# furio1999/EO_Diffusion

Hardware: AMD Instinct MI355X
Metric: denoising steps/sec (UNet fwd + DDPM update) at 256x256 bs=16 (higher is better)
Workload: dtype f32; 1 GPU; DDPM sampling step, 256x256x3, batch 16 per GPU, UNet arch A0 (base 128, mults [1,2,3,4], 1 res-block(s), attn_res []), Philox noise, x0-clipped update; global_batch=16, image_size=256, parallelism=batch-sharded x1, accumulate=fp32, precision_mode=fp32x3

## Files before the change

### eo_diffusion_amd/csrc/igemm.hip

```cpp
#include <type_traits>

#include "common.h"

struct IgemmP {
    const char* a0;
    const char* a1;
    const char* b;
    const float* bias;
    const float* cbias;
    const char* res;
    char* y;
    long long cbias_stride;
    int N, H, W, C0, C1, Cin, Cout, KS, stride, pad, ups, pad_tl, Ho, Wo, HoWo, Heff, Weff;
    int tw_log2, th;
    int tiles_pw, tiles_pi;
    long long lda, ldb, ldc, sa0, sa1, sb0, sb1, sc0, sc1;
    int nb1, bias_mode, c_f32;
    long long M;
    int Ncols, K, taps, KT, tiles_m, tiles_n, out_nchw;
    int kc0, kc1;
    int tapmajor_log2;
    int ldk;
    const float* gn_ss;
    int gn_silu;
    float* stats;
    int stats_P, tiles_per_image;
    int splitk;
    int splitk_per;
    float alpha;
    const float* w_scale;
    const int* w_rexp;
    int w_row0;
    int Hd, Wd, HWd, par, par_y, par_x;
    unsigned taplist;
    const char* sx0;
    const char* sx1;
    const char* b2;
    int SC0, SC1, skc0, skc1;
    int n_base;
    int tpw;
    const float* a_bound;
    const float* skip_bound;
    const float* b_bound;
    int ab_tab_off;
    int a_ps;
    const float* y_ps_bound;
};

template <typename T> struct Mma;
template <> struct Mma<half_t> {
    static __device__ __forceinline__ void run(const i32x4& a, const i32x4& b, f32x16& c) {
        c = __builtin_amdgcn_mfma_f32_32x32x16_f16(__builtin_bit_cast(half8, a), __builtin_bit_cast(half8, b), c, 0, 0, 0);
    }
};
template <> struct Mma<float> {
    static __device__ __forceinline__ void run(const i32x4& a, const i32x4& b, f32x16& c) {
        f32x4 af = __builtin_bit_cast(f32x4, a), bf = __builtin_bit_cast(f32x4, b);
#pragma unroll
        for (int j = 0; j < 4; ++j) c = __builtin_amdgcn_mfma_f32_32x32x2f32(af[j], bf[j], c, 0, 0, 0);
    }
};

#define EOD_SPLIT_ASCALE 16.0f
__device__ __forceinline__ void split4(const f32x4& f, int (&hi)[2], int (&lo)[2]) {
    half4 h, l;
#pragma unroll
    for (int e = 0; e < 4; ++e) {
        h[e] = (half_t)f[e];
        l[e] = (half_t)(f[e] - (float)h[e]);
    }
    const auto hb = __builtin_bit_cast(__attribute__((ext_vector_type(2))) int, h);
    const auto lb = __builtin_bit_cast(__attribute__((ext_vector_type(2))) int, l);
    hi[0] = hb[0]; hi[1] = hb[1]; lo[0] = lb[0]; lo[1] = lb[1];
}
__device__ __forceinline__ void split4_scaled(const f32x4& v, float s, int (&hi)[2], int (&lo)[2]) {
    int h01, h23, l01, l23;
    asm("v_fma_mixlo_f16 %0, %4, %5, 0\n\t"
        "v_fma_mixlo_f16 %1, %4, %7, 0\n\t"
        "v_fma_mixhi_f16 %0, %4, %6, 0\n\t"
        "v_fma_mixhi_f16 %1, %4, %8, 0\n\t"
        "v_fma_mixlo_f16 %2, %4, %5, -%0 op_sel_hi:[0,0,1]\n\t"
        "v_fma_mixlo_f16 %3, %4, %7, -%1 op_sel_hi:[0,0,1]\n\t"
        "v_fma_mixhi_f16 %2, %4, %6, -%0 op_sel:[0,0,1] op_sel_hi:[0,0,1]\n\t"
        "v_fma_mixhi_f16 %3, %4, %8, -%1 op_sel:[0,0,1] op_sel_hi:[0,0,1]"
        : "=&v"(h01), "=&v"(h23), "=&v"(l01), "=&v"(l23)
        : "v"(s), "v"(v[0]), "v"(v[1]), "v"(v[2]), "v"(v[3]));
    hi[0] = h01; hi[1] = h23; lo[0] = l01; lo[1] = l23;
}
__device__ __forceinline__ i32x4 split_pair_exchange_scaled(const f32x4& v, float s, bool odd_chunk) {
    int hi[2], lo[2];
    split4_scaled(v, s, hi, lo);
    const int s0 = odd_chunk ? hi[0] : lo[0], s1 = odd_chunk ? hi[1] : lo[1];
    const int r0 = __builtin_amdgcn_mov_dpp(s0, 0xB1, 0xF, 0xF, true), r1 = __builtin_amdgcn_mov_dpp(s1, 0xB1, 0xF, 0xF, true);
    return odd_chunk ? i32x4{r0, r1, lo[0], lo[1]} : i32x4{hi[0], hi[1], r0, r1};
}
__device__ __forceinline__ i32x4 split_pair_exchange(const f32x4& f, bool odd_chunk) {
    int hi[2], lo[2];
    split4(f, hi, lo);
    const int s0 = odd_chunk ? hi[0] : lo[0], s1 = odd_chunk ? hi[1] : lo[1];
    const int r0 = __builtin_amdgcn_mov_dpp(s0, 0xB1, 0xF, 0xF, true), r1 = __builtin_amdgcn_mov_dpp(s1, 0xB1, 0xF, 0xF, true);
    return odd_chunk ? i32x4{r0, r1, lo[0], lo[1]} : i32x4{hi[0], hi[1], r0, r1};
}

typedef __attribute__((address_space(3))) void lds_void;

#define EOD_OOB 0x80000000u
#define EOD_WINDOW 0x80000000u

__device__ __forceinline__ __amdgpu_buffer_rsrc_t make_rsrc(const void* base) {
    return __builtin_amdgcn_make_buffer_rsrc(const_cast<void*>(base), 0, (int)EOD_WINDOW, 0x00020000);
}
__device__ __forceinline__ void blds16(__amdgpu_buffer_rsrc_t rs, unsigned voff, unsigned soff, char* lds_dst_wave_uniform) {
    __builtin_amdgcn_raw_ptr_buffer_load_lds(rs, (lds_void*)lds_dst_wave_uniform, 16, voff, soff, 0, 0);
}

struct TileGeom {
    int tile_m, n_first, rem_first, ty0, tx0;
    long long offA, offB, offC;
};

template <int BM>
__device__ __forceinline__ bool decode_row(const IgemmP& p, const TileGeom& g, int r, int& nrel, int& ho, int& wo) {
    if (p.tw_log2 >= 0) {
        nrel = 0;
        ho = g.ty0 + (r >> p.tw_log2);
        wo = g.tx0 + (r & ((1 << p.tw_log2) - 1));
        const bool inside = wo < p.Wd;
        if (p.par) {
            ho = 2 * ho + p.par_y;
            wo = 2 * wo + p.par_x;
        }
        return inside;
    }
    int rem = g.rem_first + r;
    nrel = 0;
    if (rem >= p.HWd) {
        nrel = rem / p.HWd;
        rem -= nrel * p.HWd;
    }
    ho = rem / p.Wd;
    wo = rem - ho * p.Wd;
    if (p.par) {
        ho = 2 * ho + p.par_y;
        wo = 2 * wo + p.par_x;
    }
    return (long long)g.tile_m * BM + r < p.M;
}

template <bool CONV, int BM>
__device__ __forceinline__ TileGeom make_geom(const IgemmP& p, int tile_m) {
    TileGeom g = {};
    g.tile_m = tile_m;
    if constexpr (CONV) {
        if (p.tw_log2 >= 0) {
            g.n_first = tile_m / p.tiles_pi;
            const int t = tile_m - g.n_first * p.tiles_pi;
            const int ty = t / p.tiles_pw;
            g.ty0 = ty * p.th;
            g.tx0 = (t - ty * p.tiles_pw) << p.tw_log2;
        } else {
            const long long m0 = (long long)tile_m * BM;
            g.n_first = (int)(m0 / p.HWd);
            g.rem_first = (int)(m0 - (long long)g.n_first * p.HWd);
        }
    } else {
        const int z = blockIdx.y;
        const int b0 = z / p.nb1, b1 = z - b0 * p.nb1;
        g.offA = b0 * p.sa0 + b1 * p.sa1;
        g.offB = b0 * p.sb0 + b1 * p.sb1;
        g.offC = b0 * p.sc0 + b1 * p.sc1;
    }
    return g;
}

#ifdef EOD_STAMP
__device__ unsigned long long g_eod_stamp[65536][16];
#define EOD_STAMP_AT(k)                                                                    \
    do {                                                                                   \
// ... 706 lines not shown
            for (int i = 0; i < TM; ++i)
#pragma unroll
                for (int j = 0; j < TN; ++j)
                    acc[i][j] = DIRECT ? __builtin_amdgcn_mfma_f32_16x16x32_f16(__builtin_bit_cast(half8, bl[j]), __builtin_bit_cast(half8, ah[i]), acc[i][j], 0, 0, 0)
                                       : __builtin_amdgcn_mfma_f32_16x16x32_f16(__builtin_bit_cast(half8, ah[i]), __builtin_bit_cast(half8, bl[j]), acc[i][j], 0, 0, 0);
#pragma unroll
            for (int i = 0; i < TM; ++i)
#pragma unroll
                for (int j = 0; j < TN; ++j)
                    acc[i][j] = DIRECT ? __builtin_amdgcn_mfma_f32_16x16x32_f16(__builtin_bit_cast(half8, bh[j]), __builtin_bit_cast(half8, ah[i]), acc[i][j], 0, 0, 0)
                                       : __builtin_amdgcn_mfma_f32_16x16x32_f16(__builtin_bit_cast(half8, ah[i]), __builtin_bit_cast(half8, bh[j]), acc[i][j], 0, 0, 0);
            continue;
        } else if constexpr (MS == 16) {
#pragma unroll
            for (int s = 0; s < 2; ++s) {
                const int o = ((4 * s + lh) ^ sw) * 16;
                i32x4 fa16[TM], fb16[TN];
#pragma unroll
                for (int i = 0; i < TM; ++i) fa16[i] = *reinterpret_cast<const i32x4*>(sb + a_rd + i * MS * BKB + o);
#pragma unroll
                for (int j = 0; j < TN; ++j) fb16[j] = *reinterpret_cast<const i32x4*>(sb + b_rd + j * MS * BKB + o);
#pragma unroll
                for (int i = 0; i < TM; ++i)
#pragma unroll
                    for (int j = 0; j < TN; ++j)
                        acc[i][j] = __builtin_amdgcn_mfma_f32_16x16x32_f16(__builtin_bit_cast(half8, fa16[i]), __builtin_bit_cast(half8, fb16[j]), acc[i][j], 0, 0, 0);
            }
            continue;
        }
        if constexpr (MS == 32) {
        i32x4 fa[2][TM], fb[2][TN];
#pragma unroll
        for (int i = 0; i < TM; ++i) fa[0][i] = *reinterpret_cast<const i32x4*>(sb + a_rd + i * 32 * BKB + coff[0]);
#pragma unroll
        for (int j = 0; j < TN; ++j) fb[0][j] = *reinterpret_cast<const i32x4*>(sb + b_rd + j * 32 * BKB + coff[0]);
        __builtin_amdgcn_sched_group_barrier(0x100, TM + TN, 0);
#pragma unroll
        for (int s = 0; s < 4; ++s) {
            const int cur = s & 1, nx = cur ^ 1;
            if (s < 3) {
#pragma unroll
                for (int i = 0; i < TM; ++i) fa[nx][i] = *reinterpret_cast<const i32x4*>(sb + a_rd + i * 32 * BKB + coff[s + 1]);
#pragma unroll
                for (int j = 0; j < TN; ++j) fb[nx][j] = *reinterpret_cast<const i32x4*>(sb + b_rd + j * 32 * BKB + coff[s + 1]);
                __builtin_amdgcn_sched_group_barrier(0x100, TM + TN, 0);
            }
#pragma unroll
            for (int i = 0; i < TM; ++i)
#pragma unroll
                for (int j = 0; j < TN; ++j) Mma<T>::run(fa[cur][i], fb[cur][j], acc[i][j]);
            __builtin_amdgcn_sched_group_barrier(0x008, TM * TN * (sizeof(T) == 4 ? 4 : 1), 0);
        }
        }
    }
    __builtin_amdgcn_s_waitcnt(0xc07f);
    __builtin_amdgcn_s_barrier();

    if constexpr (DIRECT) {
        halo_epilogue_direct<BM, BN, WAVES_M, WAVES_N>(pe, g, acc, wave, lane, n0, pre_bq, pe.alpha, pre_we);
    } else if constexpr (sizeof(T) == 4) {
        igemm_epilogue<T, CONV, BM, BN, WAVES_M, WAVES_N, true, MS>(pe, g, acc, smem, wave, lane, n0, rowtab, rowtab_n);
    } else {
        if (CONV ? p.splitk > 1 : p.c_f32 != 0)
            igemm_epilogue<T, CONV, BM, BN, WAVES_M, WAVES_N, true, MS>(pe, g, acc, smem, wave, lane, n0);
        else
            igemm_epilogue<T, CONV, BM, BN, WAVES_M, WAVES_N, false, MS>(pe, g, acc, smem, wave, lane, n0);
    }
}

template <int TN, int MS>
__device__ __forceinline__ void prefetch_bcol(const IgemmP& p, int ncols, int col0, int lane, int n_first, float (&out)[TN]) {
    const int lr = AccLayout<MS>::col(lane);
#pragma unroll
    for (int j = 0; j < TN; ++j) {
        const int col = col0 + j * MS + lr;
        const bool ok = col < ncols;
        float v = (ok && p.bias && p.bias_mode == 1) ? p.bias[col] : 0.0f;
        if (ok && p.cbias) v += p.cbias[(long long)n_first * p.cbias_stride + col];
        out[j] = v;
    }
}

template <typename T, int BN, int WAVES_M, int WAVES_N, bool UPS, int BSTAGES, bool GN, bool SPLIT = false, int MS = 32, bool SKIP = false, bool STREAM = false,
          bool KSPLIT = false>
__global__ __launch_bounds__(64 * WAVES_M * WAVES_N, WAVES_N == 4 ? 1 : 2) void conv3x3_halo_kernel(const IgemmP p) {
    static_assert(!KSPLIT || (!STREAM && !UPS && BN == 128), "K slices: the 128-column 4-wave instances");
    static_assert(!SKIP || (MS == 16 && !UPS && WAVES_M == 2), "fused skip conv: 16x16x32 instances of the 8x16 tile");
    static_assert(!SPLIT || (sizeof(T) == 4 && MS == 16), "the split-fp16 product is a mode of fp32 storage, on 16x16x32 MFMAs");
    static_assert(MS == 32 || SPLIT || sizeof(T) == 2, "the 16x16x32 shape exists for the fp16 products only");
    constexpr bool XF = GN || SPLIT;
    constexpr bool DIRECT = SPLIT && MS == 16 && BN >= 64;
    static_assert(!STREAM || (DIRECT && !SKIP && !UPS), "streaming instances: direct epilogue, no fused skip phase");
    constexpr int NW = WAVES_M * WAVES_N;
    constexpr int BM = WAVES_N == 4 ? 64 * WAVES_M : 32 * NW, TH = BM / 16, TW = 16;
    constexpr int PH = UPS ? TH / 2 + 2 : TH + 2, PW = UPS ? TW / 2 + 2 : TW + 2, PR = PH * PW;
    constexpr int PG = (PR + 7) / 8;
    constexpr int LAH = (PG + NW - 1) / NW;
    constexpr int ES = sizeof(T), EPC = 16 / ES, BKB = 128, BK = BKB / ES;
    constexpr int WM = BM / WAVES_M, WN = BN / WAVES_N, TM = WM / MS, TN = WN / MS;
    constexpr int GB = BN / 8, LB = GB / NW;
    constexpr int ABUF = PG * 1024, BSTAGE = BN * BKB;
    static_assert(GB % NW == 0 && LAH <= 6 && BSTAGES == 2, "layout");

    extern __shared__ __attribute__((aligned(16))) char smem[];
    char* const sA = smem;
    char* const sB = smem + 2 * ABUF;
    char* const sS = sB + BSTAGES * BSTAGE;
    EOD_STAMP_AT(0);

    const int tid = threadIdx.x, lane = tid & 63;
    const int wave = __builtin_amdgcn_readfirstlane(tid >> 6);
    const int wm = wave / WAVES_N, wn = wave % WAVES_N;
    int tile_m, tile_n;
    map_tile(p, tile_m, tile_n);
    int ntile = 1;
    if constexpr (STREAM) {
        tile_m *= p.tpw;
        ntile = min(p.tpw, p.tiles_m - tile_m);
    }
    const int n0 = p.n_base + tile_n * BN;
    TileGeom g = make_geom<true, BM>(p, tile_m);
    float pre_bcol[DIRECT ? 1 : TN];
    f32x4 pre_bq[DIRECT ? TN : 1];
    int pre_we[DIRECT ? TN : 1];
    if constexpr (DIRECT) {
        prefetch_bcol4<TN>(p, p.Ncols, n0 + wn * WN, lane, g.n_first, pre_bq);
        prefetch_wexp4<TN>(p, p.Ncols, n0 + wn * WN, p.w_row0, lane, pre_we);
    } else {
        prefetch_bcol<TN, MS>(p, p.Ncols, n0 + wn * WN, lane, g.n_first, pre_bcol);
    }
    float wsc1 = 1.0f;
    if constexpr (SPLIT) wsc1 = p.w_scale[1];
    AbScale asc = {EOD_SPLIT_ASCALE, 1.0f};
    const float silu_k = p.gn_silu ? -1.44269504088896341f : 0.0f, silu_c = p.gn_silu ? 0.0f : -__builtin_inff();
    if constexpr (SPLIT) {
        if (p.a_bound) asc = ab_scale_of(ab_wave_bound(p.a_bound, g.n_first));
        if constexpr (SKIP) {
            if (p.skip_bound) {
                const AbScale k = ab_scale_of(ab_wave_bound(p.skip_bound, g.n_first));
                if (k.s < asc.s) asc = k;
            }
        }
    }

    const int srow = lane >> 3, sslot = lane & 7;
    unsigned ppix[LAH];
    const int bchunk0 = sslot ^ ((4 * wave + (srow >> 1)) & 7);
    unsigned pck = 0;
    unsigned pvalid = 0;
#pragma unroll
    for (int i = 0; i < LAH; ++i) {
        const int prow = (wave + NW * i) * 8 + srow;
        const int px = prow - (prow / PW) * PW;
        pck |= (unsigned)(sslot ^ ((px >> 1) & 7)) << (3 * i);
    }
    auto set_tile_pieces = [&](const TileGeom& tg) {
        pvalid = 0;
#pragma unroll
        for (int i = 0; i < LAH; ++i) {
            const int prow = (wave + NW * i) * 8 + srow;
            const int py = prow / PW, px = prow - py * PW;
            const int hi = (UPS ? tg.ty0 / 2 : tg.ty0) - 1 + py, wi = (UPS ? tg.tx0 / 2 : tg.tx0) - 1 + px;
            const bool ok = (wave + NW * i) < PG && prow < PR && (unsigned)hi < (unsigned)p.H && (unsigned)wi < (unsigned)p.W;
            if (ok) pvalid |= 1u << i;
            ppix[i] = (unsigned)(hi * p.W + wi);
        }
    };
    set_tile_pieces(g);
    auto pchunk_of = [&](int i) { return (int)((pck >> (3 * i)) & 7u); };
    unsigned b_v[LB];
#pragma unroll
    for (int i = 0; i < LB; ++i) {
        const int row = (wave + NW * i) * 8 + srow;
        b_v[i] = (n0 + row < p.Ncols) ? (unsigned)(row * p.Cin * ES) + bchunk0 * 16 : EOD_OOB;
    }
    const __amdgpu_buffer_rsrc_t rsA0 = make_rsrc(p.a0 + (long long)g.n_first * p.H * p.W * p.C0 * ES);
    const __amdgpu_buffer_rsrc_t rsA1 = make_rsrc(p.a1 ? p.a1 + (long long)g.n_first * p.H * p.W * p.C1 * ES : p.a0);
    const __amdgpu_buffer_rsrc_t rsB = make_rsrc(p.b + (long long)n0 * p.Cin * ES);
    const int tapstride = p.Cout * p.Cin * ES;
    __amdgpu_buffer_rsrc_t rsS = rsB;
    if constexpr (GN)
        rsS = __builtin_amdgcn_make_buffer_rsrc(const_cast<float*>(p.gn_ss) + (long long)g.n_first * p.Cin * 2, 0, p.Cin * 8, 0x00020000);

    struct Chunk {
        int src, kin, cw;
// ... 130 lines not shown
    if constexpr (MS == 16) {
        constexpr int LROW = WM / 16;
        static_assert(LROW % 2 == 0, "the UPS row split needs an even first tile row per wave");
        const int c0 = SPLIT ? 2 * ((0x2130 >> (4 * lh)) & 3) : lh, c1 = SPLIT ? c0 + 1 : 4 + lh;
#pragma unroll
        for (int dx = 0; dx < 3; ++dx) {
            const int pxc = UPS ? ((lr + dx + 1) >> 1) : lr + dx;
            const int key = (pxc >> 1) & 7;
            const int rowb = ((UPS ? (wm * LROW) >> 1 : wm * LROW) * PW + pxc) * BKB;
            acur[0][dx] = rowb + ((c0 ^ key) << 4);
            acur[1][dx] = rowb + ((c1 ^ key) << 4);
        }
    }

    const int KC = p.kc0 + p.kc1;
    int kc_begin = 0, kc_end = KC;
    if constexpr (KSPLIT) {
        kc_begin = (int)blockIdx.y * p.splitk_per;
        kc_end = (int)blockIdx.y == p.splitk - 1 ? KC : kc_begin + p.splitk_per;
    }
    const int NSTEP = (kc_end - kc_begin) * 9;
    const int TSTEP = NSTEP * ntile;
    {
        const Chunk c0 = chunk_of(kc_begin);
#pragma unroll
        for (int i = 0; i < LAH; ++i)
            if ((wave + NW * i) < PG) issue_patch_piece(i, c0, sA);
        if constexpr (GN) {
            if (wave == 0) issue_ss(c0, sS);
        }
        issue_weights(0, c0, sB);
        if constexpr (XF) {
            asm volatile("s_waitcnt vmcnt(0)" ::: "memory");
            if constexpr (GN) __builtin_amdgcn_s_barrier();
#pragma unroll
            for (int i = 0; i < LAH; ++i)
                if ((wave + NW * i) < PG) transform_piece(i, c0, sA, sS);
            __builtin_amdgcn_s_waitcnt(0xc07f);
        }
    }
    EOD_STAMP_AT(1);
    int pp1 = 0;
    int step = 0;
    int qpar = 0;
    for (int k = 0; k < ntile; ++k) {
    for (int cc = kc_begin; cc < kc_end; ++cc) {
        const Chunk cur = chunk_of(cc);
        const bool next_tile = STREAM && cc + 1 == kc_end && k + 1 < ntile;
        const bool has_next = cc + 1 < kc_end || next_tile;
        const Chunk nxt = chunk_of(cc + 1 < kc_end ? cc + 1 : (next_tile ? 0 : cc));
        if constexpr (STREAM) {
            if (next_tile) set_tile_pieces(make_geom<true, BM>(p, tile_m + k + 1));
        }
        const char* abuf = sA + qpar * ABUF;
        char* abuf_next = sA + (qpar ^ 1) * ABUF;
        weight_offsets(cur, bve);
#pragma unroll
        for (int t = 0; t < 9; ++t, ++step) {
            EOD_TSTAMP_AT(4 * t + 0);
            if (!(STREAM && t == 0 && cc == kc_begin && k > 0)) {
                if (pp1 == 0) asm volatile("s_waitcnt vmcnt(0)" ::: "memory");
                else if (pp1 == 1) asm volatile("s_waitcnt vmcnt(1)" ::: "memory");
                else asm volatile("s_waitcnt vmcnt(2)" ::: "memory");
                if constexpr (XF) __builtin_amdgcn_s_waitcnt(0xc07f);
                __builtin_amdgcn_s_barrier();
            }
            EOD_TSTAMP_AT(4 * t + 1);
            if (step + 1 < TSTEP) {
                if (t < 8) issue_weights_at(t + 1, cur, bve, sB + ((step + 1) & 1) * BSTAGE);
                else issue_weights(0, nxt, sB + ((step + 1) & 1) * BSTAGE);
            }
            pp1 = 0;
            if (t < LAH && has_next && (wave + NW * t) < PG) {
                issue_patch_piece(t, nxt, abuf_next);
                pp1 = 1;
            }
            if constexpr (GN) {
                if (t == 0 && has_next && wave == 0) {
                    issue_ss(nxt, sS + (qpar ^ 1) * 1024);
                    ++pp1;
                }
            }
            EOD_TSTAMP_AT(4 * t + 2);
            const int dy = t / 3, dx = t - dy * 3;
            const char* bst = sB + (step & 1) * BSTAGE;
            int arow[TM], asw[TM];
#pragma unroll
            for (int i = 0; i < TM; ++i) {
                const int pxc = UPS ? ((pxo[i] + dx + 1) >> 1) : pxo[i] + dx;
                const int prow = UPS ? ((pyo[i] + dy + 1) >> 1) * PW + pxc : prow0[i] + dy * PW + dx;
                arow[i] = prow * BKB;
                asw[i] = (pxc >> 1) & 7;
            }
            if constexpr (MS == 16 && SPLIT) {
                const int ch = 2 * ((0x2130 >> (4 * lh)) & 3);
                i32x4 ah[TM], al[TM], bh[TN], bl[TN];
#pragma unroll
                for (int i = 0; i < TM; ++i) al[i] = *reinterpret_cast<const i32x4*>(sA + acur[1][dx] + aimm(i, dy));
#pragma unroll
                for (int j = 0; j < TN; ++j) bh[j] = *reinterpret_cast<const i32x4*>(bst + b_rd + j * MS * BKB + ((ch ^ bsw) << 4));
#pragma unroll
                for (int i = 0; i < TM; ++i) ah[i] = *reinterpret_cast<const i32x4*>(sA + acur[0][dx] + aimm(i, dy));
#pragma unroll
                for (int i = 0; i < TM; ++i)
#pragma unroll
                    for (int j = 0; j < TN; ++j)
                        acc[i][j] = DIRECT ? __builtin_amdgcn_mfma_f32_16x16x32_f16(__builtin_bit_cast(half8, bh[j]), __builtin_bit_cast(half8, al[i]), acc[i][j], 0, 0, 0)
                                           : __builtin_amdgcn_mfma_f32_16x16x32_f16(__builtin_bit_cast(half8, al[i]), __builtin_bit_cast(half8, bh[j]), acc[i][j], 0, 0, 0);
#pragma unroll
                for (int j = 0; j < TN; ++j) bl[j] = *reinterpret_cast<const i32x4*>(bst + b_rd + j * MS * BKB + (((ch + 1) ^ bsw) << 4));
#pragma unroll
                for (int i = 0; i < TM; ++i)
#pragma unroll
                    for (int j = 0; j < TN; ++j)
                        acc[i][j] = DIRECT ? __builtin_amdgcn_mfma_f32_16x16x32_f16(__builtin_bit_cast(half8, bl[j]), __builtin_bit_cast(half8, ah[i]), acc[i][j], 0, 0, 0)
                                           : __builtin_amdgcn_mfma_f32_16x16x32_f16(__builtin_bit_cast(half8, ah[i]), __builtin_bit_cast(half8, bl[j]), acc[i][j], 0, 0, 0);
#pragma unroll
                for (int i = 0; i < TM; ++i)
#pragma unroll
                    for (int j = 0; j < TN; ++j)
                        acc[i][j] = DIRECT ? __builtin_amdgcn_mfma_f32_16x16x32_f16(__builtin_bit_cast(half8, bh[j]), __builtin_bit_cast(half8, ah[i]), acc[i][j], 0, 0, 0)
                                           : __builtin_amdgcn_mfma_f32_16x16x32_f16(__builtin_bit_cast(half8, ah[i]), __builtin_bit_cast(half8, bh[j]), acc[i][j], 0, 0, 0);
            } else if constexpr (MS == 16) {
#pragma unroll
                for (int s = 0; s < 2; ++s) {
                    const int ch = 4 * s + lh;
                    i32x4 fa16[TM], fb16[TN];
#pragma unroll
                    for (int i = 0; i < TM; ++i) fa16[i] = *reinterpret_cast<const i32x4*>(sA + acur[s][dx] + aimm(i, dy));
#pragma unroll
                    for (int j = 0; j < TN; ++j) fb16[j] = *reinterpret_cast<const i32x4*>(bst + b_rd + j * MS * BKB + ((ch ^ bsw) << 4));
#pragma unroll
                    for (int i = 0; i < TM; ++i)
#pragma unroll
                        for (int j = 0; j < TN; ++j)
                            acc[i][j] = __builtin_amdgcn_mfma_f32_16x16x32_f16(__builtin_bit_cast(half8, fa16[i]), __builtin_bit_cast(half8, fb16[j]), acc[i][j], 0, 0, 0);
                }
            } else {
            i32x4 fa[2][TM], fb[2][TN];
#pragma unroll
            for (int i = 0; i < TM; ++i)
                fa[0][i] = *reinterpret_cast<const i32x4*>(abuf + arow[i] + (((0 + lh) ^ asw[i]) << 4));
#pragma unroll
            for (int j = 0; j < TN; ++j) fb[0][j] = *reinterpret_cast<const i32x4*>(bst + b_rd + j * 32 * BKB + bcoff[0]);
            __builtin_amdgcn_sched_group_barrier(0x100, TM + TN, 0);
#pragma unroll
            for (int s = 0; s < 4; ++s) {
                const int cur = s & 1, nx = cur ^ 1;
                if (s < 3) {
#pragma unroll
                    for (int i = 0; i < TM; ++i)
                        fa[nx][i] = *reinterpret_cast<const i32x4*>(abuf + arow[i] + (((2 * (s + 1) + lh) ^ asw[i]) << 4));
#pragma unroll
                    for (int j = 0; j < TN; ++j)
                        fb[nx][j] = *reinterpret_cast<const i32x4*>(bst + b_rd + j * 32 * BKB + bcoff[s + 1]);
                    __builtin_amdgcn_sched_group_barrier(0x100, TM + TN, 0);
                }
#pragma unroll
                for (int i = 0; i < TM; ++i)
#pragma unroll
                    for (int j = 0; j < TN; ++j) Mma<T>::run(fa[cur][i], fb[cur][j], acc[i][j]);
                __builtin_amdgcn_sched_group_barrier(0x008, TM * TN * (sizeof(T) == 4 ? 4 : 1), 0);
            }
            }
            EOD_TSTAMP_AT(4 * t + 3);
            if constexpr (XF) {
                if (t >= 2 && t - 2 < LAH && has_next && (wave + NW * (t - 2)) < PG)
                    transform_piece(t - 2, nxt, abuf_next, sS + (qpar ^ 1) * 1024);
            }
        }
        EOD_TSTAMP_AT(36);
#ifdef EOD_TSTAMP
        if (GN && wave == 1 && cc == 1 && k == 0 && blockIdx.x < 2048) {
            __builtin_amdgcn_s_waitcnt(0xc07f);
            if (lane < 37) g_eod_tstamp[blockIdx.x][lane] = reinterpret_cast<const unsigned long long*>(sA + ABUF + PR * 128)[lane];
        }
#endif
        if constexpr (MS == 16) {
            const int flip = qpar ? -ABUF : ABUF;
#pragma unroll
            for (int dx = 0; dx < 3; ++dx) {
                acur[0][dx] += flip;
                acur[1][dx] += flip;
            }
        }
        qpar ^= 1;
    }
    if constexpr (SKIP) {
      if (!KSPLIT || (int)blockIdx.y == p.splitk - 1) {
        constexpr int LA = BM / 8 / NW;
        constexpr int STG_A = BM * BKB, STG = STG_A + BSTAGE;
        static_assert(2 * STG <= 2 * ABUF + BSTAGES * BSTAGE, "the skip phase reuses the operand ring");
        __builtin_amdgcn_s_waitcnt(0xc07f);
        __builtin_amdgcn_s_barrier();
        const int SC = p.SC0 + p.SC1;
        const __amdgpu_buffer_rsrc_t rsX0 = make_rsrc(p.sx0 + (long long)g.n_first * p.H * p.W * p.SC0 * ES);
        const __amdgpu_buffer_rsrc_t rsX1 = make_rsrc(p.sx1 ? p.sx1 + (long long)g.n_first * p.H * p.W * p.SC1 * ES : p.sx0);
        const __amdgpu_buffer_rsrc_t rsW2 = make_rsrc(p.b2 + (long long)n0 * SC * ES);
        unsigned xpix[LA], wv[LB];
        unsigned xok = 0;
#pragma unroll
        for (int i = 0; i < LA; ++i) {
            const int row = (wave + NW * i) * 8 + srow;
            xpix[i] = (unsigned)((g.ty0 + (row >> 4)) * p.W + g.tx0 + (row & 15));
            if (g.tx0 + (row & 15) < p.W) xok |= 1u << i;
        }
#pragma unroll
        for (int i = 0; i < LB; ++i) {
            const int row = (wave + NW * i) * 8 + srow;
            wv[i] = (n0 + row < p.Ncols) ? (unsigned)(row * SC * ES) + bchunk0 * 16 : EOD_OOB;
        }
        auto issue_skip = [&](int kt, char* stg) {
            const int src = kt >= p.skc0 ? 1 : 0;
            const int kin = (src ? kt - p.skc0 : kt) * BK, cw = src ? p.SC1 : p.SC0;
            const bool ktail = kin + BK > cw;
#pragma unroll
            for (int i = 0; i < LA; ++i) {
                unsigned v = ((xok >> i) & 1u) ? xpix[i] * (unsigned)(cw * ES) + bchunk0 * 16 : EOD_OOB;
                if (ktail) v = (kin + bchunk0 * EPC < cw) ? v : EOD_OOB;
                if (src)
                    blds16(rsX1, v, (unsigned)(kin * ES), stg + (wave + NW * i) * 1024);
                else
                    blds16(rsX0, v, (unsigned)(kin * ES), stg + (wave + NW * i) * 1024);
            }
#pragma unroll
            for (int i = 0; i < LB; ++i) {
                unsigned v = wv[i];
                if (ktail) v = (kin + (SPLIT ? (bchunk0 >> 1) * 8 : bchunk0 * EPC) < cw) ? v : EOD_OOB;
                blds16(rsW2, v, (unsigned)(((src ? p.SC0 : 0) + kin) * ES), stg + STG_A + (wave + NW * i) * 1024);
            }
        };
        const int KS = p.skc0 + p.skc1;
        const int a_rd = (wm * WM + lr) * BKB;
        const int b_rd2 = STG_A + (wn * WN + lr) * BKB;
        if (KS > 0) issue_skip(0, smem);
        for (int kt = 0; kt < KS; ++kt) {
            char* stg = smem + (kt & 1) * STG;
            asm volatile("s_waitcnt vmcnt(0)" ::: "memory");
            if constexpr (SPLIT) {
#pragma unroll
                for (int i = 0; i < LA; ++i) {
                    char* ptr = stg + (wave + NW * i) * 1024 + lane * 16;
                    const f32x4 f = *reinterpret_cast<const f32x4*>(ptr);
                    *reinterpret_cast<i32x4*>(ptr) = split_pair_exchange_scaled(f, asc.s, (bchunk0 & 1) != 0);
                }
                __builtin_amdgcn_s_waitcnt(0xc07f);
            }
            __builtin_amdgcn_s_barrier();
            if (kt + 1 < KS) issue_skip(kt + 1, smem + ((kt + 1) & 1) * STG);
            if constexpr (SPLIT) {
                const int ch = 2 * ((0x2130 >> (4 * lh)) & 3);
// ... 1035 lines not shown
    EOD_CHECK_LAUNCH("conv_head");
    return EOD_OK;
}

template <typename T>
__global__ void splitk_reduce_kernel(const float* __restrict__ ws, int S, long long M, int Cout, int HoWo, float alpha,
                                     const float* __restrict__ bias, const float* __restrict__ cbias, long long cbias_stride,
                                     const T* __restrict__ res, T* __restrict__ y, const float* __restrict__ w_scale) {
    if (w_scale) alpha *= w_scale[1];
    const long long total4 = M * Cout / 4;
    for (long long i = (long long)blockIdx.x * blockDim.x + threadIdx.x; i < total4; i += (long long)gridDim.x * blockDim.x) {
        const long long e = i * 4, m = e / Cout;
        const int c = (int)(e - m * Cout);
        f32x4 a = {0.f, 0.f, 0.f, 0.f};
        for (int z = 0; z < S; ++z) a += *reinterpret_cast<const f32x4*>(ws + (long long)z * M * Cout + e);
        const long long n = m / HoWo;
#pragma unroll
        for (int k = 0; k < 4; ++k) {
            float v = a[k] * alpha;
            if (bias) v += bias[c + k];
            if (cbias) v += cbias[n * cbias_stride + c + k];
            if (res) v += (float)res[e + k];
            y[e + k] = (T)v;
        }
    }
}

template <typename T>
__global__ __launch_bounds__(256) void splitk_reduce_stats_kernel(const float* __restrict__ ws, int S, long long M, int Cout, int HoWo, float alpha,
                                                                  const float* __restrict__ bias, const float* __restrict__ cbias,
                                                                  long long cbias_stride, const T* __restrict__ res, T* __restrict__ y,
                                                                  float* __restrict__ stats) {
    __shared__ float red[16][16][8];
    const int tx = threadIdx.x & 15, ty = threadIdx.x >> 4, n = blockIdx.y;
    const int c = (blockIdx.x * 16 + tx) * 4;
    float ss[4] = {0.f, 0.f, 0.f, 0.f}, sq[4] = {0.f, 0.f, 0.f, 0.f};
    if (c < Cout) {
        float b4[4];
#pragma unroll
        for (int k = 0; k < 4; ++k) b4[k] = (bias ? bias[c + k] : 0.0f) + (cbias ? cbias[(long long)n * cbias_stride + c + k] : 0.0f);
        const long long zs = M * Cout;
        for (int pix = ty; pix < HoWo; pix += 16) {
            const long long e = ((long long)n * HoWo + pix) * Cout + c;
            f32x4 a = {0.f, 0.f, 0.f, 0.f};
            int z = 0;
            for (; z + 4 <= S; z += 4) {
                const f32x4 v0 = *reinterpret_cast<const f32x4*>(ws + (long long)z * zs + e), v1 = *reinterpret_cast<const f32x4*>(ws + (long long)(z + 1) * zs + e);
                const f32x4 v2 = *reinterpret_cast<const f32x4*>(ws + (long long)(z + 2) * zs + e), v3 = *reinterpret_cast<const f32x4*>(ws + (long long)(z + 3) * zs + e);
                a += v0; a += v1; a += v2; a += v3;
            }
            for (; z < S; ++z) a += *reinterpret_cast<const f32x4*>(ws + (long long)z * zs + e);
#pragma unroll
            for (int k = 0; k < 4; ++k) {
                float v = a[k] * alpha + b4[k];
                if (res) v += (float)res[e + k];
                const T o = (T)v;
                y[e + k] = o;
                const float x = (float)o;
                ss[k] += x;
                sq[k] += x * x;
            }
        }
    }
#pragma unroll
    for (int k = 0; k < 4; ++k) {
        red[ty][tx][2 * k] = ss[k];
        red[ty][tx][2 * k + 1] = sq[k];
    }
    __syncthreads();
    if (ty == 0 && c < Cout) {
        float* dst = stats + ((long long)n * Cout + c) * 2;
#pragma unroll
        for (int k = 0; k < 8; ++k) {
            float t = 0.0f;
#pragma unroll
            for (int r = 0; r < 16; ++r) t += red[r][tx][k];
            dst[k] = t;
        }
    }
}

#include <stdlib.h>
#include <string.h>
enum { OPT_SKIP_FUSE, OPT_HEAD, OPT_HALO_BN256, OPT_GN_FUSE_MAX_COUT, OPT_HALO_TPW, OPT_HALO_SPLITK, OPT_FIRST, OPT_HEAD_TPW, OPT_S2_HALO, OPT_COUNT };
static const char* const g_opt_name[OPT_COUNT] = {"skip_fuse", "head", "halo_bn256", "gn_fuse_max_cout", "halo_tpw", "halo_splitk", "first", "head_tpw",
                                                  "s2_halo"};
static const char* const g_opt_env[OPT_COUNT] = {"EOD_SKIP_FUSE", "EOD_HEAD", "EOD_HALO_BN256", "EOD_GN_FUSE_MAX_COUT", "EOD_HALO_TPW", "EOD_HALO_SPLITK",
                                                 "EOD_FIRST", "EOD_HEAD_TPW", "EOD_S2_HALO"};
static int g_opt[OPT_COUNT] = {1, 1, 1, -1, 1, 1, 1, 0, 1};
static bool g_opt_init = false;
static int opt(int k) {
    if (!g_opt_init) {
        for (int i = 0; i < OPT_COUNT; ++i) {
            const char* e = getenv(g_opt_env[i]);
            if (e) g_opt[i] = atoi(e);
        }
        g_opt_init = true;
    }
    return g_opt[k];
}
extern "C" int eod_set_option(const char* name, int value) {
    (void)opt(0);
    for (int i = 0; name && i < OPT_COUNT; ++i)
        if (!strcmp(name, g_opt_name[i])) {
            const int prev = g_opt[i];
            g_opt[i] = value;
            return prev;
        }
    eod_set_error("set_option: unknown option '%s'", name ? name : "(null)");
    return EOD_EINVAL;
}
extern "C" int eod_get_option(const char* name) {
    (void)opt(0);
    for (int i = 0; name && i < OPT_COUNT; ++i)
        if (!strcmp(name, g_opt_name[i])) return g_opt[i];
    eod_set_error("get_option: unknown option '%s'", name ? name : "(null)");
    return EOD_EINVAL;
}

template <typename T, bool CONV, int BM, int BN, int WAVES_M, int WAVES_N, int STAGES, bool SPLIT = false, int MS = 32, bool DIRECT = false>
static int launch_cfg(IgemmP& p, int batch, hipStream_t st) {
    constexpr int BK = 128 / (int)sizeof(T);
    constexpr int WM = BM / WAVES_M, WN = BN / WAVES_N, NW = WAVES_M * WAVES_N;
    const size_t ring = STAGES * (size_t)(BM + BN) * 128;
    const size_t epi = NW * (size_t)WM * (WN + 4) * sizeof(float);
    size_t lds = ring > epi ? ring : epi;
    if (SPLIT && CONV) {
        lds = (lds + 15) & ~(size_t)15;
        p.ab_tab_off = (int)lds;
        lds += (BM + 2) * 2 * sizeof(float);
    }
    auto kern = igemm_kernel<T, CONV, BM, BN, WAVES_M, WAVES_N, STAGES, SPLIT, MS, DIRECT>;
    static bool attr_done = false;
    if (!attr_done) {
        (void)hipFuncSetAttribute(reinterpret_cast<const void*>(kern), hipFuncAttributeMaxDynamicSharedMemorySize, (int)lds);
        attr_done = true;
    }
    if (CONV) {
        p.kc0 = (p.C0 + BK - 1) / BK;
        p.kc1 = (p.C1 + BK - 1) / BK;
        p.KT = (p.kc0 + p.kc1) * p.taps;
        if (p.tapmajor_log2 >= 0) p.KT = (9 * p.C0 + BK - 1) / BK;
    } else {
        p.KT = (p.K + BK - 1) / BK;
    }
    p.tiles_n = (p.Ncols + BN - 1) / BN;
    p.tw_log2 = -1;
    if (CONV) {
        int tw = 16;
        while (tw > p.Wd) tw >>= 1;
        if (tw >= 4 && p.Wd % tw == 0 && (BM % tw) == 0 && p.Hd % (BM / tw) == 0) {
            int l = 0;
            while ((1 << l) < tw) ++l;
            p.tw_log2 = l;
            p.th = BM / tw;
            p.tiles_pw = p.Wd / tw;
            p.tiles_pi = p.tiles_pw * (p.Hd / p.th);
            p.tiles_m = p.tiles_pi * p.N;
        } else {
            p.tiles_m = (int)((p.M + BM - 1) / BM);
        }
    } else {
        p.tiles_m = (int)((p.M + BM - 1) / BM);
    }
    const long long nblk = (long long)p.tiles_m * p.tiles_n;
    if (nblk <= 0 || nblk > 0x7fffffffLL) {
        eod_set_error("igemm: bad grid %lld", nblk);
        return EOD_EINVAL;
    }
    hipLaunchKernelGGL(kern, dim3((unsigned)nblk, (unsigned)batch), dim3(64 * NW), lds, st, p);
    EOD_CHECK_LAUNCH("igemm");
    return EOD_OK;
}

template <typename T, int BN, int WAVES_M, int WAVES_N, bool UPS, int BSTAGES, bool GN, bool SPLIT = false, int MS = 32, bool SKIP = false, bool STREAM = false,
          bool KSPLIT = false>
static int launch_halo(IgemmP& p, hipStream_t st) {
    if constexpr (!KSPLIT && !STREAM && !UPS && BN == 128 && WAVES_N == 2) {
        if (p.splitk > 1) return launch_halo<T, BN, WAVES_M, WAVES_N, UPS, BSTAGES, GN, SPLIT, MS, SKIP, false, true>(p, st);
    }
    if constexpr (!KSPLIT) {
        if (p.splitk > 1) {
            eod_set_error("conv_halo: K slices exist for the 128-column 4-wave instances only");
            return EOD_EINVAL;
        }
    }
    constexpr int BK = 128 / (int)sizeof(T);
    constexpr int NW = WAVES_M * WAVES_N, BM = WAVES_N == 4 ? 64 * WAVES_M : 32 * NW, TH = BM / 16;
    constexpr int WM = BM / WAVES_M, WN = BN / WAVES_N;
    constexpr int PR = UPS ? (TH / 2 + 2) * 10 : (TH + 2) * 18, PG = (PR + 7) / 8;
    const size_t ring = 2 * (size_t)(PG * 1024) + BSTAGES * (size_t)BN * 128 + (GN ? 2048 : 0);
    const size_t epi = NW * (size_t)WM * (WN + 4) * sizeof(float);
    const size_t lds = ring > epi ? ring : epi;
    auto kern = conv3x3_halo_kernel<T, BN, WAVES_M, WAVES_N, UPS, BSTAGES, GN, SPLIT, MS, SKIP, STREAM, KSPLIT>;
    if constexpr (SKIP) {
        p.skc0 = (p.SC0 + BK - 1) / BK;
        p.skc1 = (p.SC1 + BK - 1) / BK;
    }
    static bool attr_done = false;
    if (!attr_done) {
        (void)hipFuncSetAttribute(reinterpret_cast<const void*>(kern), hipFuncAttributeMaxDynamicSharedMemorySize, (int)lds);
        attr_done = true;
    }
    p.kc0 = (p.C0 + BK - 1) / BK;
    p.kc1 = (p.C1 + BK - 1) / BK;
    p.KT = (p.kc0 + p.kc1) * 9;
    p.tiles_n = (p.Ncols - p.n_base + BN - 1) / BN;
    p.tw_log2 = 4;
    p.th = TH;
    p.tiles_pw = (p.Wo + 15) / 16;
    p.tiles_pi = p.tiles_pw * (p.Ho / TH);
    p.tiles_m = p.tiles_pi * p.N;
    p.tiles_per_image = p.tiles_pi;
    p.tpw = 1;
    if constexpr (SPLIT && MS == 16 && BN >= 128 && !SKIP && !UPS) {
        const long long slots = 256LL * (NW == 4 ? 2 : 1);
        int want = opt(OPT_HALO_TPW);
        if (want <= 0) {
            want = 1;
            while (want < 8 && (long long)p.tiles_m * p.tiles_n / (2 * want) >= 2 * slots) want *= 2;
        }
        while (want > 1 && p.tiles_pi % want) --want;
        if (p.splitk > 1) want = 1;
        if constexpr (!STREAM) {
            if (want > 1) return launch_halo<T, BN, WAVES_M, WAVES_N, UPS, BSTAGES, GN, SPLIT, MS, SKIP, true>(p, st);
        } else {
            p.tpw = want;
        }
    }
    const long long nblk = (long long)(p.tiles_m / p.tpw) * p.tiles_n;
    if (nblk <= 0 || nblk > 0x7fffffffLL) {
        eod_set_error("conv_halo: bad grid %lld", nblk);
        return EOD_EINVAL;
    }
    hipLaunchKernelGGL(kern, dim3((unsigned)nblk, (unsigned)(p.splitk > 1 ? p.splitk : 1)), dim3(64 * NW), lds, st, p);
    EOD_CHECK_LAUNCH("conv3x3_halo");
    return EOD_OK;
}

template <typename T, bool CONV> static int launch_T(IgemmP& p, int batch, hipStream_t st) {
    if constexpr (sizeof(T) == 2) {
        if (p.Ncols <= 32) return launch_cfg<T, CONV, 128, 32, 4, 1, 2, false, 16>(p, batch, st);
        if (p.Ncols <= 64) return launch_cfg<T, CONV, 128, 64, 4, 1, 2, false, 16>(p, batch, st);
        return launch_cfg<T, CONV, 128, 128, 2, 2, 2, false, 16>(p, batch, st);
    } else {
        if (p.Ncols <= 32) return launch_cfg<T, CONV, 128, 32, 4, 1, 2>(p, batch, st);
        if (p.Ncols <= 64) return launch_cfg<T, CONV, 128, 64, 4, 1, 2>(p, batch, st);
        return launch_cfg<T, CONV, 128, 128, 2, 2, 2>(p, batch, st);
    }
}

static int launch_conv_split(IgemmP& p, int batch, hipStream_t st) {
    if (p.Ncols <= 32) return launch_cfg<float, true, 128, 32, 4, 1, 2, true, 16>(p, batch, st);
    if (p.Ncols <= 64) return launch_cfg<float, true, 128, 64, 4, 1, 2, true, 16>(p, batch, st);
    const bool direct = p.splitk <= 1 && !p.out_nchw && p.HWd % 128 == 0 && p.M % 128 == 0 && !p.par && p.Ncols % 4 == 0;
    if (p.Ncols % 256 == 0 && batch == 1 && ((p.M + 127) / 128) * (p.Ncols / 256) >= 256 && opt(OPT_HALO_BN256))
        return direct ? launch_cfg<float, true, 128, 256, 2, 4, 2, true, 16, true>(p, batch, st)
                      : launch_cfg<float, true, 128, 256, 2, 4, 2, true, 16>(p, batch, st);
    return direct ? launch_cfg<float, true, 128, 128, 2, 2, 2, true, 16, true>(p, batch, st)
                  : launch_cfg<float, true, 128, 128, 2, 2, 2, true, 16>(p, batch, st);
}

extern "C" int eod_conv_tapmajor_ldk(int C0, int dtype) {
    const int bk = 128 / (dtype == EOD_F16 ? 2 : 4);
    return (9 * C0 + bk - 1) / bk * bk;
}

static bool conv_uses_halo(const eod_conv_desc* d, int Ho, int Wo) {
    const bool shape_ok = ((d->Cout > 64 && !d->out_nchw_f32) || (d->Cout <= 32 && d->out_nchw_f32 && !d->upsample)) && d->upsample != 2;
    const bool w_ok = Wo % 16 == 0 || (Wo == 8 && d->Cout > 64 && !d->out_nchw_f32 && !d->upsample);
    return d->ksize == 3 && d->stride == 1 && d->pad == 1 && !d->pad_tl && w_ok && Ho % 8 == 0 && shape_ok && !d->w_tapmajor;
}
static int conv_waves_m(const eod_conv_desc* d, bool halo) { return (halo || d->Cout > 64) ? 2 : 4; }
static int conv_bm(const eod_conv_desc* d, bool halo) { return 128; }

static bool conv_split_ok(const eod_conv_desc* d, int Ho, int Wo) {
    return d->dtype == EOD_F32 && (d->w_tapmajor || (d->C0 % 8 == 0 && d->C1 % 8 == 0)) && d->upsample != 2;
}
static bool conv_parity_ok(const eod_conv_desc* d, int Ho, int Wo) {
    return d->upsample == 2 && d->ksize == 3 && d->stride == 1 && d->pad == 1 && !d->pad_tl && !d->out_nchw_f32 && !d->stats &&
           !d->w_tapmajor && !d->w_split && Ho % 2 == 0 && Wo % 2 == 0;
}
static bool conv_up4_ok(const eod_conv_desc* d) {
    const bool store_ok = d->dtype == EOD_F16 || (d->dtype == EOD_F32 && d->w_split);
    return d->upsample == 3 && d->ksize == 3 && d->stride == 1 && d->pad == 1 && !d->pad_tl && d->C1 == 0 && !d->x2 && d->Cout > 64 &&
           d->Cout % 8 == 0 && d->C0 % 8 == 0 && (d->W % 16 == 0 || d->W == 8) && d->H % 8 == 0 && !d->out_nchw_f32 && !d->w_tapmajor &&
           !d->gn_scale_shift && store_ok;
}
extern "C" int eod_conv_up4_ok(const eod_conv_desc* d) { return d && conv_up4_ok(d) ? 1 : 0; }
static bool conv_up4_bwd_ok(const eod_conv_desc* d) {
    return d->upsample == 4 && d->dtype == EOD_F16 && d->ksize == 3 && d->stride == 1 && d->pad == 1 && !d->pad_tl && d->C1 == 0 && !d->x2 &&
           d->Cout > 64 && d->Cout % 8 == 0 && d->C0 % 8 == 0 && d->H % 2 == 0 && d->W % 2 == 0 && d->Ho == d->H / 2 && d->Wo == d->W / 2 &&
           d->Wo % 16 == 0 && d->Ho % 8 == 0 && !d->out_nchw_f32 && !d->w_tapmajor && !d->gn_scale_shift && !d->stats && !d->w_split;
}
extern "C" int eod_conv_up4_bwd_ok(const eod_conv_desc* d) { return d && conv_up4_bwd_ok(d) ? 1 : 0; }
static int conv_up4_bwd(const eod_conv_desc* d, void* stream) {
    EOD_REQUIRE(d->N > 0 && d->H > 0 && d->W > 0 && d->C0 > 0 && d->Cout > 0 && d->x && d->w && d->y, "conv (upsample 4): bad args");
    EOD_REQUIRE(conv_up4_bwd_ok(d), "conv: upsample = 4 needs a geometry for which eod_conv_up4_bwd_ok(d) == 1");
    EOD_REQUIRE(eod_aligned16(d->x) && eod_aligned16(d->w), "conv: 16-byte alignment");
    EOD_REQUIRE((long long)d->H * d->W * d->C0 * 2 < 0x7fffffffLL && 9LL * d->Cout * 4 * d->C0 * 2 < 0x7fffffffLL, "conv (upsample 4): operand exceeds the 2 GiB window");
    IgemmP p = {};
    p.a0 = (const char*)d->x; p.b = (const char*)d->w; p.bias = d->bias; p.bias_mode = d->bias ? 1 : 0;
    p.cbias = d->cbias; p.cbias_stride = d->cbias_stride; p.res = (const char*)d->res; p.y = (char*)d->y;
    p.N = d->N; p.H = d->Ho; p.W = d->Wo;
    p.C0 = d->C0; p.C1 = 0; p.Cin = d->C0; p.Cout = d->Cout; p.KS = 3; p.stride = 1; p.pad = 1;
    p.Ho = d->Ho; p.Wo = d->Wo; p.HoWo = d->Ho * d->Wo; p.Heff = d->Ho; p.Weff = d->Wo;
    p.Hd = d->Ho; p.Wd = d->Wo; p.HWd = d->Ho * d->Wo;
    p.M = (long long)d->N * d->Ho * d->Wo; p.Ncols = d->Cout; p.taps = 9; p.alpha = d->alpha; p.nb1 = 1; p.tapmajor_log2 = -1;
// ... 426 lines not shown
```

Baseline: 39.88 steps/s.

## Interleave GroupNorm-SiLU patch transform with MFMAs via inline asm in halo conv

Adds a hand-scheduled inline-assembly block that interleaves the GroupNorm scale/shift, SiLU (exp/rcp) and fp16 hi/lo split of the next patch with the 16x16x32 MFMA chain of the current tap. Previously this transform ran after the MFMA loop. The block is enabled by default through a new option for the GN-fused split-fp32 halo instances with 64x64 wave tiles. The goal is to hide the VALU transform latency under matrix-core work. The costs are more template instances and register pressure, plus a fixed s_nop and asm volatile that constrain compiler scheduling.

```diff
diff --git a/eo_diffusion_amd/csrc/igemm.hip b/eo_diffusion_amd/csrc/igemm.hip
--- a/eo_diffusion_amd/csrc/igemm.hip
+++ b/eo_diffusion_amd/csrc/igemm.hip
@@ -87,13 +87,55 @@
         : "v"(s), "v"(v[0]), "v"(v[1]), "v"(v[2]), "v"(v[3]));
     hi[0] = h01; hi[1] = h23; lo[0] = l01; lo[1] = l23;
 }
+__device__ __forceinline__ i32x4 pair_exchange(const int (&hi)[2], const int (&lo)[2], bool odd_chunk) {
+    const int s0 = odd_chunk ? hi[0] : lo[0], s1 = odd_chunk ? hi[1] : lo[1];
+    const int r0 = __builtin_amdgcn_mov_dpp(s0, 0xB1, 0xF, 0xF, true), r1 = __builtin_amdgcn_mov_dpp(s1, 0xB1, 0xF, 0xF, true);
+    return odd_chunk ? i32x4{r0, r1, lo[0], lo[1]} : i32x4{hi[0], hi[1], r0, r1};
+}
 __device__ __forceinline__ i32x4 split_pair_exchange_scaled(const f32x4& v, float s, bool odd_chunk) {
     int hi[2], lo[2];
     split4_scaled(v, s, hi, lo);
-    const int s0 = odd_chunk ? hi[0] : lo[0], s1 = odd_chunk ? hi[1] : lo[1];
-    const int r0 = __builtin_amdgcn_mov_dpp(s0, 0xB1, 0xF, 0xF, true), r1 = __builtin_amdgcn_mov_dpp(s1, 0xB1, 0xF, 0xF, true);
-    return odd_chunk ? i32x4{r0, r1, lo[0], lo[1]} : i32x4{hi[0], hi[1], r0, r1};
-}
+    return pair_exchange(hi, lo, odd_chunk);
+}
+#define EOD_HALO_ASM_BLOCK(MIXHI, MIXLO)                  \
+    "v_fma_f32 %4, %18, %19, %20\n\t"                     \
+    "v_fma_f32 %5, %4, %21, %22\n\t"                      \
+    "v_mfma_f32_16x16x32_f16 %0, %8, %16, %0\n\t"         \
+    "v_exp_f32 %5, %5\n\t"                                \
+    "v_mfma_f32_16x16x32_f16 %1, %9, %16, %1\n\t"         \
+    "v_add_f32 %5, 1.0, %5\n\t"                           \
+    "v_mfma_f32_16x16x32_f16 %2, %10, %16, %2\n\t"        \
+    "v_rcp_f32 %5, %5\n\t"                                \
+    "v_mfma_f32_16x16x32_f16 %3, %11, %16, %3\n\t"        \
+    "v_mul_f32 %5, %4, %5\n\t"                            \
+    "v_mfma_f32_16x16x32_f16 %0, %12, %17, %0\n\t"        \
+    MIXHI "\n\t"                                          \
+    "v_mfma_f32_16x16x32_f16 %1, %13, %17, %1\n\t"        \
+    MIXLO "\n\t"                                          \
+    "v_mfma_f32_16x16x32_f16 %2, %14, %17, %2\n\t"        \
+    "v_mfma_f32_16x16x32_f16 %3, %15, %17, %3\n\t"        \
+    "v_mfma_f32_16x16x32_f16 %0, %8, %17, %0\n\t"         \
+    "v_mfma_f32_16x16x32_f16 %1, %9, %17, %1\n\t"         \
+    "v_mfma_f32_16x16x32_f16 %2, %10, %17, %2\n\t"        \
+    "v_mfma_f32_16x16x32_f16 %3, %11, %17, %3\n\t"        \
+    "s_nop 7"
+template <bool ODD>
+__device__ __forceinline__ void halo_asm_block(f32x4 (&acc)[4], const i32x4 (&bh)[4], const i32x4 (&bl)[4], const i32x4& al, const i32x4& ah,
+                                               float x, float sc, float sh, float k, float c, float s, int& hi, int& lo) {
+    float t0, t1;
+    if constexpr (ODD) {
+        asm volatile(EOD_HALO_ASM_BLOCK("v_fma_mixhi_f16 %6, %23, %5, 0", "v_fma_mixhi_f16 %7, %23, %5, -%6 op_sel:[0,0,1] op_sel_hi:[0,0,1]")
+                     : "+v"(acc[0]), "+v"(acc[1]), "+v"(acc[2]), "+v"(acc[3]), "=&v"(t0), "=&v"(t1), "+v"(hi), "+v"(lo)
+                     : "v"(bh[0]), "v"(bh[1]), "v"(bh[2]), "v"(bh[3]), "v"(bl[0]), "v"(bl[1]), "v"(bl[2]), "v"(bl[3]), "v"(al), "v"(ah),
+                       "v"(x), "v"(sc), "v"(sh), "s"(k), "v"(c), "v"(s));
+    } else {
+        asm volatile(EOD_HALO_ASM_BLOCK("v_fma_mixlo_f16 %6, %23, %5, 0", "v_fma_mixlo_f16 %7, %23, %5, -%6 op_sel_hi:[0,0,1]")
+                     : "+v"(acc[0]), "+v"(acc[1]), "+v"(acc[2]), "+v"(acc[3]), "=&v"(t0), "=&v"(t1), "=&v"(hi), "=&v"(lo)
+                     : "v"(bh[0]), "v"(bh[1]), "v"(bh[2]), "v"(bh[3]), "v"(bl[0]), "v"(bl[1]), "v"(bl[2]), "v"(bl[3]), "v"(al), "v"(ah),
+                       "v"(x), "v"(sc), "v"(sh), "s"(k), "v"(c), "v"(s));
+    }
+}
+#undef EOD_HALO_ASM_BLOCK
 __device__ __forceinline__ i32x4 split_pair_exchange(const f32x4& f, bool odd_chunk) {
     int hi[2], lo[2];
     split4(f, hi, lo);
@@ -966,7 +1008,7 @@
 }
 
 template <typename T, int BN, int WAVES_M, int WAVES_N, bool UPS, int BSTAGES, bool GN, bool SPLIT = false, int MS = 32, bool SKIP = false, bool STREAM = false,
-          bool KSPLIT = false>
+          bool KSPLIT = false, bool HASM = false>
 __global__ __launch_bounds__(64 * WAVES_M * WAVES_N, WAVES_N == 4 ? 1 : 2) void conv3x3_halo_kernel(const IgemmP p) {
     static_assert(!KSPLIT || (!STREAM && !UPS && BN == 128), "K slices: the 128-column 4-wave instances");
     static_assert(!SKIP || (MS == 16 && !UPS && WAVES_M == 2), "fused skip conv: 16x16x32 instances of the 8x16 tile");
@@ -985,6 +1027,7 @@
     constexpr int GB = BN / 8, LB = GB / NW;
     constexpr int ABUF = PG * 1024, BSTAGE = BN * BKB;
     static_assert(GB % NW == 0 && LAH <= 6 && BSTAGES == 2, "layout");
+    static_assert(!HASM || (GN && SPLIT && DIRECT && !UPS && TM == 4 && TN == 4), "halo_asm: fp32x3 GroupNorm-fused 64 x 64 wave tiles");
 
     extern __shared__ __attribute__((aligned(16))) char smem[];
     char* const sA = smem;
@@ -1281,6 +1324,8 @@
                 }
             }
             EOD_TSTAMP_AT(4 * t + 2);
+            const bool xf_now = t >= 2 && t - 2 < LAH && has_next && (wave + NW * (t - 2)) < PG;
+            bool xf_done = false;
             const int dy = t / 3, dx = t - dy * 3;
             const char* bst = sB + (step & 1) * BSTAGE;
             int arow[TM], asw[TM];
@@ -1294,6 +1339,40 @@
             if constexpr (MS == 16 && SPLIT) {
                 const int ch = 2 * ((0x2130 >> (4 * lh)) & 3);
                 i32x4 ah[TM], al[TM], bh[TN], bl[TN];
+                if constexpr (HASM) {
+                    if (xf_now) {
+                        const int xi = t - 2;
+                        XfPre pre;
+                        xf_load(xi, abuf_next, sS + (qpar ^ 1) * 1024, pre);
+#pragma unroll
+                        for (int j = 0; j < TN; ++j) bh[j] = *reinterpret_cast<const i32x4*>(bst + b_rd + j * MS * BKB + ((ch ^ bsw) << 4));
+#pragma unroll
+                        for (int j = 0; j < TN; ++j) bl[j] = *reinterpret_cast<const i32x4*>(bst + b_rd + j * MS * BKB + (((ch + 1) ^ bsw) << 4));
+                        al[0] = *reinterpret_cast<const i32x4*>(sA + acur[1][dx] + aimm(0, dy));
+                        ah[0] = *reinterpret_cast<const i32x4*>(sA + acur[0][dx] + aimm(0, dy));
+                        const int pc = pchunk_of(xi);
+                        const bool ok = ((pvalid >> xi) & 1u) && (!nxt.ktail || (nxt.kin + pc * EPC < nxt.cw));
+                        const float sl = ok ? asc.s : 0.0f;
+                        const f32x4 f = __builtin_bit_cast(f32x4, pre.raw);
+                        const f32x4 q0 = pre.q[0], q1 = pre.q[1];
+                        const float sc[4] = {q0[0], q0[2], q1[0], q1[2]}, sh[4] = {q0[1], q0[3], q1[1], q1[3]};
+                        int hi[2], lo[2];
+#pragma unroll
+                        for (int i = 0; i < TM; ++i) {
+                            if (i + 1 < TM) {
+                                al[i + 1] = *reinterpret_cast<const i32x4*>(sA + acur[1][dx] + aimm(i + 1, dy));
+                                ah[i + 1] = *reinterpret_cast<const i32x4*>(sA + acur[0][dx] + aimm(i + 1, dy));
+                            }
+                            if (i & 1)
+                                halo_asm_block<true>(acc[i], bh, bl, al[i], ah[i], f[i], sc[i], sh[i], silu_k, silu_c, sl, hi[i >> 1], lo[i >> 1]);
+                            else
+                                halo_asm_block<false>(acc[i], bh, bl, al[i], ah[i], f[i], sc[i], sh[i], silu_k, silu_c, sl, hi[i >> 1], lo[i >> 1]);
+                        }
+                        *reinterpret_cast<i32x4*>(abuf_next + (wave + NW * xi) * 1024 + lane * 16) = pair_exchange(hi, lo, (pc & 1) != 0);
+                        xf_done = true;
+                    }
+                }
+                if (!xf_done) {
 #pragma unroll
                 for (int i = 0; i < TM; ++i) al[i] = *reinterpret_cast<const i32x4*>(sA + acur[1][dx] + aimm(i, dy));
 #pragma unroll
@@ -1320,6 +1399,7 @@
                     for (int j = 0; j < TN; ++j)
                         acc[i][j] = DIRECT ? __builtin_amdgcn_mfma_f32_16x16x32_f16(__builtin_bit_cast(half8, bh[j]), __builtin_bit_cast(half8, ah[i]), acc[i][j], 0, 0, 0)
                                            : __builtin_amdgcn_mfma_f32_16x16x32_f16(__builtin_bit_cast(half8, ah[i]), __builtin_bit_cast(half8, bh[j]), acc[i][j], 0, 0, 0);
+                }
             } else if constexpr (MS == 16) {
 #pragma unroll
                 for (int s = 0; s < 2; ++s) {
@@ -1364,8 +1444,7 @@
             }
             EOD_TSTAMP_AT(4 * t + 3);
             if constexpr (XF) {
-                if (t >= 2 && t - 2 < LAH && has_next && (wave + NW * (t - 2)) < PG)
-                    transform_piece(t - 2, nxt, abuf_next, sS + (qpar ^ 1) * 1024);
+                if (xf_now && !xf_done) transform_piece(t - 2, nxt, abuf_next, sS + (qpar ^ 1) * 1024);
             }
         }
         EOD_TSTAMP_AT(36);
@@ -2567,12 +2646,13 @@
 
 #include <stdlib.h>
 #include <string.h>
-enum { OPT_SKIP_FUSE, OPT_HEAD, OPT_HALO_BN256, OPT_GN_FUSE_MAX_COUT, OPT_HALO_TPW, OPT_HALO_SPLITK, OPT_FIRST, OPT_HEAD_TPW, OPT_S2_HALO, OPT_COUNT };
+enum { OPT_SKIP_FUSE, OPT_HEAD, OPT_HALO_BN256, OPT_GN_FUSE_MAX_COUT, OPT_HALO_TPW, OPT_HALO_SPLITK, OPT_FIRST, OPT_HEAD_TPW, OPT_S2_HALO, OPT_HALO_ASM,
+       OPT_COUNT };
 static const char* const g_opt_name[OPT_COUNT] = {"skip_fuse", "head", "halo_bn256", "gn_fuse_max_cout", "halo_tpw", "halo_splitk", "first", "head_tpw",
-                                                  "s2_halo"};
+                                                  "s2_halo", "halo_asm"};
 static const char* const g_opt_env[OPT_COUNT] = {"EOD_SKIP_FUSE", "EOD_HEAD", "EOD_HALO_BN256", "EOD_GN_FUSE_MAX_COUT", "EOD_HALO_TPW", "EOD_HALO_SPLITK",
-                                                 "EOD_FIRST", "EOD_HEAD_TPW", "EOD_S2_HALO"};
-static int g_opt[OPT_COUNT] = {1, 1, 1, -1, 1, 1, 1, 0, 1};
+                                                 "EOD_FIRST", "EOD_HEAD_TPW", "EOD_S2_HALO", "EOD_HALO_ASM"};
+static int g_opt[OPT_COUNT] = {1, 1, 1, -1, 1, 1, 1, 0, 1, 1};
 static bool g_opt_init = false;
 static int opt(int k) {
     if (!g_opt_init) {
@@ -2659,10 +2739,14 @@
 }
 
 template <typename T, int BN, int WAVES_M, int WAVES_N, bool UPS, int BSTAGES, bool GN, bool SPLIT = false, int MS = 32, bool SKIP = false, bool STREAM = false,
-          bool KSPLIT = false>
+          bool KSPLIT = false, bool HASM = false>
 static int launch_halo(IgemmP& p, hipStream_t st) {
+    constexpr bool ASM_OK = GN && SPLIT && MS == 16 && !UPS && ((BN == 128 && WAVES_N == 2) || (BN == 256 && WAVES_N == 4));
+    if constexpr (ASM_OK && !HASM) {
+        if (opt(OPT_HALO_ASM)) return launch_halo<T, BN, WAVES_M, WAVES_N, UPS, BSTAGES, GN, SPLIT, MS, SKIP, STREAM, KSPLIT, true>(p, st);
+    }
     if constexpr (!KSPLIT && !STREAM && !UPS && BN == 128 && WAVES_N == 2) {
-        if (p.splitk > 1) return launch_halo<T, BN, WAVES_M, WAVES_N, UPS, BSTAGES, GN, SPLIT, MS, SKIP, false, true>(p, st);
+        if (p.splitk > 1) return launch_halo<T, BN, WAVES_M, WAVES_N, UPS, BSTAGES, GN, SPLIT, MS, SKIP, false, true, HASM>(p, st);
     }
     if constexpr (!KSPLIT) {
         if (p.splitk > 1) {
@@ -2677,7 +2761,7 @@
     const size_t ring = 2 * (size_t)(PG * 1024) + BSTAGES * (size_t)BN * 128 + (GN ? 2048 : 0);
     const size_t epi = NW * (size_t)WM * (WN + 4) * sizeof(float);
     const size_t lds = ring > epi ? ring : epi;
-    auto kern = conv3x3_halo_kernel<T, BN, WAVES_M, WAVES_N, UPS, BSTAGES, GN, SPLIT, MS, SKIP, STREAM, KSPLIT>;
+    auto kern = conv3x3_halo_kernel<T, BN, WAVES_M, WAVES_N, UPS, BSTAGES, GN, SPLIT, MS, SKIP, STREAM, KSPLIT, HASM>;
     if constexpr (SKIP) {
         p.skc0 = (p.SC0 + BK - 1) / BK;
         p.skc1 = (p.SC1 + BK - 1) / BK;
@@ -2708,7 +2792,7 @@
         while (want > 1 && p.tiles_pi % want) --want;
         if (p.splitk > 1) want = 1;
         if constexpr (!STREAM) {
-            if (want > 1) return launch_halo<T, BN, WAVES_M, WAVES_N, UPS, BSTAGES, GN, SPLIT, MS, SKIP, true>(p, st);
+            if (want > 1) return launch_halo<T, BN, WAVES_M, WAVES_N, UPS, BSTAGES, GN, SPLIT, MS, SKIP, true, false, HASM>(p, st);
         } else {
             p.tpw = want;
         }
```

Result: slower. 38.27 steps/s, median of 2 (-4.0%).
